# joyecnu/STTODE

Hardware: AMD Instinct MI355X
Metric: predicted-trajectories/sec (20-sample best-of-K) (higher is better)
Workload: dtype f32

## Files before the change

### sttode_amd/csrc/chain32.hip

```cpp
#include "chain.hpp"
#include "latency_bodies.hpp"
#include "frontend_body.hpp"
#include "api_util.hpp"
#include "../../include/sttode_hip.h"
#include <cstdlib>
#include <cstddef>

#ifdef C32_DIAG_TRACE
__shared__ long long g_tr_ph[4];
#define C32_TRACE_BEGIN() long long _tr_t0 = 0, _tr_c0 = 0; if (threadIdx.x == 0 && A.dbg) { _tr_t0 = __builtin_amdgcn_s_memrealtime(); _tr_c0 = __builtin_amdgcn_s_memtime(); }
#define C32_TRACE_END(kind) do { if (threadIdx.x == 0 && A.dbg) { \
        const long long _t1 = __builtin_amdgcn_s_memrealtime(); unsigned _hw, _xcc; \
        asm volatile("s_getreg_b32 %0, hwreg(HW_REG_HW_ID)" : "=s"(_hw)); asm volatile("s_getreg_b32 %0, hwreg(HW_REG_XCC_ID)" : "=s"(_xcc)); \
        const unsigned long long _r = atomicAdd((unsigned long long*)A.dbg, 1ull); if ((long long)_r >= A.dbg[1]) break;  \
        long long* _p = A.dbg + 8 + _r * 12; _p[0] = A.trace_tag; _p[1] = blockIdx.x; _p[2] = (kind); _p[3] = _tr_t0; _p[4] = _t1; _p[5] = _hw; _p[6] = _xcc; \
        _p[8] = g_tr_ph[0]; _p[9] = g_tr_ph[1]; _p[10] = g_tr_ph[2]; _p[7] = __builtin_amdgcn_s_memtime() - _tr_c0; _p[11] = g_tr_ph[3]; } } while (0)
#define C32_TRACE_PHASE(i) do { if (threadIdx.x == 0) g_tr_ph[i] = __builtin_amdgcn_s_memrealtime(); } while (0)
#else
#define C32_TRACE_PHASE(i) do { } while (0)
#define C32_TRACE_BEGIN() do { } while (0)
#define C32_TRACE_END(kind) do { } while (0)
#endif

#include "role_body.hpp"
// ... 186 lines not shown
        asm volatile("s_waitcnt lgkmcnt(0)" ::: "memory");
#endif
        par ^= 1;
        fetched = false;
        __builtin_amdgcn_sched_barrier(0);
    }
};
typedef ChainStreamT<C32_CMAX * C32_TILE, false> ChainStream;

__device__ __forceinline__ void tile_mma(f32x16& acc, const f32x4* __restrict__ t, const f32x16& B) {
#pragma unroll
    for (int g = 0; g < 4; ++g) {
        const f32x4 a = t[g * 64];
#pragma unroll
        for (int r = 0; r < 4; ++r) acc = __builtin_amdgcn_mfma_f32_32x32x2f32(a[r], B[4 * g + r], acc, 0, 0, 0);
    }
}

__device__ __forceinline__ void gather_rows(const void* base, unsigned voff, unsigned slot_addr) {
    glds16_sv<0>(base, voff, slot_addr);
    glds16_sv<32>(base, voff, slot_addr + 1024);
    glds16_sv<64>(base, voff, slot_addr + 2048);
    glds16_sv<96>(base, voff, slot_addr + 3072);
}
__device__ __forceinline__ unsigned row_off(int row, int width, int h) { return (unsigned)row * (unsigned)(width * 4) + (unsigned)h * 16; }

struct Frag { f32x4 a[4]; };
__device__ __forceinline__ void ldfrag(Frag& f, const f32x4* __restrict__ t) {
#pragma unroll
    for (int g = 0; g < 4; ++g) f.a[g] = t[g * 64];
}
__device__ __forceinline__ void tile_mma2(f32x16& acc, const Frag& cur, const f32x16& B, Frag& nxt, const f32x4* __restrict__ tn) {
#pragma unroll
    for (int g = 0; g < 4; ++g) {
        if (g == 2 && tn) {
            ldfrag(nxt, tn);
            __builtin_amdgcn_sched_barrier(0);
        }
#pragma unroll
        for (int r = 0; r < 4; ++r) acc = __builtin_amdgcn_mfma_f32_32x32x2f32(cur.a[g][r], B[4 * g + r], acc, 0, 0, 0);
    }
}

template <class ST>
__device__ __forceinline__ void tile_mma2f(ST& st, f32x16& acc, const Frag& cur, const f32x16& B, Frag& nxt, const f32x4* __restrict__ tn, int nf = 1) {
#pragma unroll
    for (int g = 0; g < 4; ++g) {
        if (g == 2) {
            __builtin_amdgcn_sched_barrier(0);
            if (nf >= 1) st.fetch();
            if (nf >= 2) st.fetch_more();
            if (tn) ldfrag(nxt, tn);
            __builtin_amdgcn_sched_barrier(0);
        }
#pragma unroll
        for (int r = 0; r < 4; ++r) acc = __builtin_amdgcn_mfma_f32_32x32x2f32(cur.a[g][r], B[4 * g + r], acc, 0, 0, 0);
    }
}

template <int KH, class ST>
__device__ __forceinline__ void mlp_l12(ST& st, const f32x4* slot, const f32x4* zslot, const f32x16* Bh, const float* tab, unsigned aoff,
                                        const float* tab_next, unsigned aoff_next, f32x16 (&acc2)[8], int lane) {
    const unsigned slot_addr = __builtin_amdgcn_readfirstlane(lds_addr(slot));
    constexpr int KT1 = 1 + KH;
    static_assert((KT1 + 8) % 3 == 0, "hidden tile must be a whole number of chunks");
#pragma unroll
    for (int R = 0; R < 8; ++R) acc2[R] = splat16(0.f);
#pragma unroll 1
    for (int ht = 0; ht < 16; ++ht) {
        f32x16 h1, zb;
#pragma unroll
        for (int a = 0; a < 4; ++a) {
            const f32x4 v = slot[a * 64 + lane];
            h1[4 * a + 0] = v[0]; h1[4 * a + 1] = v[1]; h1[4 * a + 2] = v[2]; h1[4 * a + 3] = v[3];
        }
#pragma unroll
        for (int a = 0; a < 4; ++a) {
            const f32x4 v = zslot[a * 64 + lane];
            zb[4 * a + 0] = v[0]; zb[4 * a + 1] = v[1]; zb[4 * a + 2] = v[2]; zb[4 * a + 3] = v[3];
        }
        asm volatile("s_waitcnt lgkmcnt(0)" ::: "memory");
        __builtin_amdgcn_sched_barrier(0);
        const bool nl = ht + 1 < 16;
        const void* nb = nl ? (const void*)(reinterpret_cast<const char*>(tab) + 128 * (ht + 1)) : (const void*)tab_next;
        const unsigned no = nl ? aoff : aoff_next;
        Frag fr[2];
#pragma unroll
        for (int i = 0; i < KT1 + 8; ++i) {
            if (i % 3 == 0) {
                if (i > 0) st.end();
                ldfrag(fr[i & 1], st.cur());
                st.begin(3);
                if (i == 0) {
#ifndef C32_DIAG_NOGATHER
                    gather_rows(nb, no, slot_addr);
#endif
                    __builtin_amdgcn_sched_barrier(0);
                }
            }
            const f32x4* tn = (i % 3 < 2) ? st.cur() + (i % 3 + 1) * C32_TILE : nullptr;
            if (i == 0) {
                tile_mma2f(st, h1, fr[i & 1], zb, fr[(i + 1) & 1], tn);
            } else if (i < KT1) {
                if (i % 3 == 0) tile_mma2f(st, h1, fr[i & 1], Bh[i - 1], fr[(i + 1) & 1], tn);
                else tile_mma2(h1, fr[i & 1], Bh[i - 1], fr[(i + 1) & 1], tn);
            } else {
                if (i == KT1) h1 = relu16(h1);
                if (i % 3 == 0) tile_mma2f(st, acc2[i - KT1], fr[i & 1], h1, fr[(i + 1) & 1], tn);
                else tile_mma2(acc2[i - KT1], fr[i & 1], h1, fr[(i + 1) & 1], tn);
            }
        }
        st.end();
    }
}

template <int NO, int NEXT = 0, class ST>
__device__ __forceinline__ void mlp_l3(ST& st, f32x16 (&acc2)[8], const float* __restrict__ b2, const float* __restrict__ b3,
                                       f32x16 (&out)[NO], int h) {
#pragma unroll
    for (int R = 0; R < 8; ++R) {
        STT_FENCE();
        const f32x16 b = ldrows(b2 + 32 * R, h);
        acc2[R] = relu16(acc2[R] + b);
        asm volatile("" : "+v"(acc2[R]));
    }
    STT_FENCE();
#pragma unroll
    for (int o = 0; o < NO; ++o) out[o] = ldrows(b3 + 32 * o, h);
    Frag fr[2];
#pragma unroll
    for (int i = 0; i < 8 * NO; ++i) {
        if (i % 3 == 0) {
            if (i > 0) st.end();
            ldfrag(fr[i & 1], st.cur());
            const int left = 8 * NO - (i + 3);
            st.begin(left >= 3 ? 3 : left > 0 ? left : NEXT);
        }
        const f32x4* tn = (i % 3 < 2 && i + 1 < 8 * NO) ? st.cur() + (i % 3 + 1) * C32_TILE : nullptr;
        if (i % 3 == 0) tile_mma2f(st, out[i / 8], fr[i & 1], acc2[i % 8], fr[(i + 1) & 1], tn);
        else tile_mma2(out[i / 8], fr[i & 1], acc2[i % 8], fr[(i + 1) & 1], tn);
    }
    st.end();
}

typedef __bf16 bf16x8 __attribute__((ext_vector_type(8)));
typedef __bf16 bf16x2 __attribute__((ext_vector_type(2)));
typedef float f32x2v __attribute__((ext_vector_type(2)));
typedef unsigned u32x4v __attribute__((ext_vector_type(4)));
#define C32_TILE_B3 384
#define C32_BUF_B3 (C32_CMAX * C32_TILE_B3)
struct B3 { bf16x8 p[3][2]; };
__device__ __forceinline__ float bf_lo(unsigned u) { return __uint_as_float(u << 16); }
__device__ __forceinline__ float bf_hi(unsigned u) { return __uint_as_float(u & 0xffff0000u); }
__device__ __forceinline__ void split3(const f32x16& x, B3& o) {
#pragma unroll
    for (int kb = 0; kb < 2; ++kb) {
        unsigned hi[4], mi[4], lo[4];
#pragma unroll
        for (int q = 0; q < 4; ++q) {
            const float x0 = x[8 * kb + 2 * q], x1 = x[8 * kb + 2 * q + 1];
            const f32x2v v = {x0, x1};
            hi[q] = __builtin_bit_cast(unsigned, __builtin_convertvector(v, bf16x2));
            const float r0 = x0 - bf_lo(hi[q]), r1 = x1 - bf_hi(hi[q]);
            const f32x2v rv = {r0, r1};
            mi[q] = __builtin_bit_cast(unsigned, __builtin_convertvector(rv, bf16x2));
            const f32x2v qv = {r0 - bf_lo(mi[q]), r1 - bf_hi(mi[q])};
            lo[q] = __builtin_bit_cast(unsigned, __builtin_convertvector(qv, bf16x2));
        }
        const u32x4v H = {hi[0], hi[1], hi[2], hi[3]}, M = {mi[0], mi[1], mi[2], mi[3]}, L = {lo[0], lo[1], lo[2], lo[3]};
        o.p[0][kb] = __builtin_bit_cast(bf16x8, H);
        o.p[1][kb] = __builtin_bit_cast(bf16x8, M);
        o.p[2][kb] = __builtin_bit_cast(bf16x8, L);
    }
}
struct Frag6 { f32x4 a[6]; };
__device__ __forceinline__ void ldfrag6(Frag6& f, const f32x4* __restrict__ t) {
#pragma unroll
    for (int i = 0; i < 6; ++i) f.a[i] = t[i * 64];
}
__device__ __forceinline__ void tile_mma_b3(f32x16& acc, const Frag6& cur, const B3& B, Frag6& nxt, const f32x4* __restrict__ tn) {
#pragma unroll
    for (int kb = 0; kb < 2; ++kb) {
        if (kb == 1 && tn) {
            ldfrag6(nxt, tn);
            __builtin_amdgcn_sched_barrier(0);
        }
        const bf16x8 ah = __builtin_bit_cast(bf16x8, cur.a[kb * 3 + 0]), am = __builtin_bit_cast(bf16x8, cur.a[kb * 3 + 1]),
                     al = __builtin_bit_cast(bf16x8, cur.a[kb * 3 + 2]);
        acc = __builtin_amdgcn_mfma_f32_32x32x16_bf16(al, B.p[0][kb], acc, 0, 0, 0);
        acc = __builtin_amdgcn_mfma_f32_32x32x16_bf16(ah, B.p[2][kb], acc, 0, 0, 0);
        acc = __builtin_amdgcn_mfma_f32_32x32x16_bf16(am, B.p[1][kb], acc, 0, 0, 0);
        acc = __builtin_amdgcn_mfma_f32_32x32x16_bf16(am, B.p[0][kb], acc, 0, 0, 0);
        acc = __builtin_amdgcn_mfma_f32_32x32x16_bf16(ah, B.p[1][kb], acc, 0, 0, 0);
        acc = __builtin_amdgcn_mfma_f32_32x32x16_bf16(ah, B.p[0][kb], acc, 0, 0, 0);
    }
}
__device__ __forceinline__ void tile_mma_b3n(f32x16& acc, const f32x4* __restrict__ t, const B3& B) {
    Frag6 f, dummy;
    ldfrag6(f, t);
    tile_mma_b3(acc, f, B, dummy, nullptr);
}
template <int KH, bool PRE, class ST>
__device__ __forceinline__ void mlp_l12_b3(ST& st, const f32x4* slot, const f32x4* zslot, const f32x16* Bh, const float* tab, unsigned aoff,
                                           const float* tab_next, unsigned aoff_next, f32x16 (&acc2)[8], int lane) {
    const unsigned slot_addr = __builtin_amdgcn_readfirstlane(lds_addr(slot));
    constexpr int KT1 = 1 + KH;
    static_assert((KT1 + 8) % 3 == 0, "hidden tile must be a whole number of chunks");
#pragma unroll
    for (int R = 0; R < 8; ++R) acc2[R] = splat16(0.f);
    B3 Bz;
    if (KH == 0) {
        f32x16 zb;
#pragma unroll
        for (int a = 0; a < 4; ++a) {
            const f32x4 v = zslot[a * 64 + lane];
            zb[4 * a + 0] = v[0]; zb[4 * a + 1] = v[1]; zb[4 * a + 2] = v[2]; zb[4 * a + 3] = v[3];
        }
        split3(zb, Bz);
    }
#pragma unroll 1
    for (int ht = 0; ht < 16; ++ht) {
        f32x16 h1;
#pragma unroll
        for (int a = 0; a < 4; ++a) {
            const f32x4 v = slot[a * 64 + lane];
            h1[4 * a + 0] = v[0]; h1[4 * a + 1] = v[1]; h1[4 * a + 2] = v[2]; h1[4 * a + 3] = v[3];
        }
        B3 Bt;
        if (KH == 0) {
            Bt = Bz;
        } else {
            f32x16 zb;
#pragma unroll
            for (int a = 0; a < 4; ++a) {
                const f32x4 v = zslot[a * 64 + lane];
                zb[4 * a + 0] = v[0]; zb[4 * a + 1] = v[1]; zb[4 * a + 2] = v[2]; zb[4 * a + 3] = v[3];
            }
            split3(zb, Bt);
        }
        asm volatile("s_waitcnt lgkmcnt(0)" ::: "memory");
        __builtin_amdgcn_sched_barrier(0);
        const bool nl = ht + 1 < 16;
        const void* nb = nl ? (const void*)(reinterpret_cast<const char*>(tab) + 128 * (ht + 1)) : (const void*)tab_next;
        const unsigned no = nl ? aoff : aoff_next;
        Frag6 fr[2];
#pragma unroll
        for (int i = 0; i < KT1 + 8; ++i) {
            if (i % 3 == 0) {
                if (i > 0) st.end();
                if (PRE) ldfrag6(fr[i & 1], st.cur());
                st.begin();
                if (i == 0) {
#ifndef C32_DIAG_NOGATHER
                    gather_rows(nb, no, slot_addr);
#endif
                    __builtin_amdgcn_sched_barrier(0);
                }
            }
            const f32x4* tc = st.cur() + (i % 3) * C32_TILE_B3;
            const f32x4* tn = (i % 3 < 2) ? tc + C32_TILE_B3 : nullptr;
            if (i > 0 && i < KT1) {
                STT_FENCE();
                split3(Bh[i - 1], Bt);
            }
            f32x16& acc = i < KT1 ? h1 : acc2[i < KT1 ? 0 : i - KT1];
            if (PRE) tile_mma_b3(acc, fr[i & 1], Bt, fr[(i + 1) & 1], tn);
            else tile_mma_b3n(acc, tc, Bt);
            if (i == KT1 - 1) {
                h1 = relu16(h1);
                split3(h1, Bt);
            }
        }
        st.end();
    }
}
template <int NO, class ST>
__device__ __forceinline__ void mlp_l3_b3(ST& st, f32x16 (&acc2)[8], const float* __restrict__ b2, const float* __restrict__ b3,
                                          f32x16 (&out)[NO], int h) {
#pragma unroll
    for (int o = 0; o < NO; ++o) out[o] = ldrows(b3 + 32 * o, h);
    Frag6 fr[2];
    B3 Bt;
#pragma unroll
    for (int i = 0; i < 8 * NO; ++i) {
        if (i % NO == 0) {
            STT_FENCE();
            const f32x16 b = ldrows(b2 + 32 * (i / NO), h);
            const f32x16 a = relu16(acc2[i / NO] + b);
            split3(a, Bt);
        }
        if (i % 3 == 0) {
            if (i > 0) st.end();
            ldfrag6(fr[i & 1], st.cur());
            st.begin();
        }
        const f32x4* tn = (i % 3 < 2 && i + 1 < 8 * NO) ? st.cur() + (i % 3 + 1) * C32_TILE_B3 : nullptr;
        tile_mma_b3(out[i % NO], fr[i & 1], Bt, fr[(i + 1) & 1], tn);
    }
    st.end();
}

__device__ __forceinline__ f32x16 b3_to_f32(const B3& b) {
    f32x16 r;
#pragma unroll
    for (int kb = 0; kb < 2; ++kb) {
        const u32x4v H = __builtin_bit_cast(u32x4v, b.p[0][kb]), M = __builtin_bit_cast(u32x4v, b.p[1][kb]), L = __builtin_bit_cast(u32x4v, b.p[2][kb]);
#pragma unroll
        for (int q = 0; q < 4; ++q) {
            r[8 * kb + 2 * q] = (bf_lo(H[q]) + bf_lo(M[q])) + bf_lo(L[q]);
            r[8 * kb + 2 * q + 1] = (bf_hi(H[q]) + bf_hi(M[q])) + bf_hi(L[q]);
        }
    }
    return r;
}
template <class ST>
__device__ __forceinline__ void gru32_steps_b3(ST& st, const float* gb, const float* cb, const f32x16& d, f32x16 (&hs)[3], int Tp, int h) {
    B3 dB, hB[3];
    split3(d, dB);
#pragma unroll
    for (int j = 0; j < 3; ++j) split3(hs[j], hB[j]);
    constexpr int T = C32_TILE_B3;
#pragma unroll 1
    for (int t = 0; t < Tp; ++t) {
        B3 eB;
        {
            f32x16 e = ldrows(cb, h);
            st.begin();
            tile_mma_b3n(e, st.cur(), dB);
            e = relu16(e);
            st.end();
            split3(e, eB);
        }
        f32x16 hn[3];
#pragma unroll
        for (int j = 0; j < 3; ++j) {
            STT_FENCE();
            f32x16 ar = ldrows(gb + 0 * 96 + 32 * j, h);
            st.begin();
            tile_mma_b3n(ar, st.cur(), eB);
            tile_mma_b3n(ar, st.cur() + T, hB[0]);
            tile_mma_b3n(ar, st.cur() + 2 * T, hB[1]);
            st.end(); st.begin();
            tile_mma_b3n(ar, st.cur(), hB[2]);
#pragma unroll
            for (int r = 0; r < 16; ++r) ar[r] = C32_SIG(ar[r]);
            STT_FENCE();
            f32x16 az = ldrows(gb + 1 * 96 + 32 * j, h);
            tile_mma_b3n(az, st.cur() + T, eB);
            tile_mma_b3n(az, st.cur() + 2 * T, hB[0]);
            st.end(); st.begin();
            tile_mma_b3n(az, st.cur(), hB[1]);
            tile_mma_b3n(az, st.cur() + T, hB[2]);
#pragma unroll
            for (int r = 0; r < 16; ++r) az[r] = C32_SIG(az[r]);
            STT_FENCE();
            f32x16 an = ldrows(gb + 3 * 96 + 32 * j, h);
            tile_mma_b3n(an, st.cur() + 2 * T, hB[0]);
            st.end(); st.begin();
            tile_mma_b3n(an, st.cur(), hB[1]);
            tile_mma_b3n(an, st.cur() + T, hB[2]);
            {
                const f32x16 bi = ldrows(gb + 2 * 96 + 32 * j, h);
#pragma unroll
                for (int r = 0; r < 16; ++r) an[r] = fmaf(ar[r], an[r], bi[r]);
            }
            STT_FENCE();
            tile_mma_b3n(an, st.cur() + 2 * T, eB);
            st.end();
            const f32x16 hp = b3_to_f32(hB[j]);
#pragma unroll
            for (int r = 0; r < 16; ++r) {
                const float ng = C32_TANH(an[r]);
                hn[j][r] = fmaf(az[r], hp[r] - ng, ng);
            }
        }
#pragma unroll
        for (int j = 0; j < 3; ++j) {
            hs[j] = hn[j];
            split3(hn[j], hB[j]);
        }
    }
}

template <bool ZS, class ST>
__device__ __forceinline__ f32x16 gru32_conv(ST& st, const float* cb, const f32x16& d, int t, int Tp, int h, bool pre) {
    f32x16 e = ldrows(cb, h);
    Frag fa, fb;
    if (ZS) {
        const int k0 = 2 * t - 2, k1 = 2 * t + 3;
        const int g0 = (k0 > 0 ? k0 : 0) >> 3, g1 = (k1 < 2 * Tp - 1 ? k1 : 2 * Tp - 1) >> 3;
        const f32x4* tc = st.cur();
#pragma unroll
        for (int g = 0; g < 4; ++g)
            if (g >= g0 && g <= g1) fa.a[g] = tc[g * 64];
        st.begin(3);
#pragma unroll
        for (int g = 0; g < 4; ++g)
            if (g >= g0 && g <= g1)
#pragma unroll
                for (int r = 0; r < 4; ++r) e = __builtin_amdgcn_mfma_f32_32x32x2f32(fa.a[g][r], d[4 * g + r], e, 0, 0, 0);
        __builtin_amdgcn_sched_barrier(0);
        if (pre) st.take_prefetched();
        else st.fetch();
    } else {
        ldfrag(fa, st.cur());
        st.begin(3);
        tile_mma2f(st, e, fa, d, fb, nullptr, pre ? 0 : 1);
        if (pre) st.take_prefetched();
    }
    e = relu16(e);
    st.end();
    return e;
}

template <bool ZS, class ST>
__device__ __forceinline__ void gru32_steps(ST& st, const float* gb, const float* cb, const f32x16& d, f32x16 (&hs)[3], int Tp, int h) {
    if (ZS) {
        const f32x16 e = gru32_conv<ZS>(st, cb, d, 0, Tp, h, false);
        Frag fa, fb;
#pragma unroll
        for (int j = 0; j < 3; ++j) {
            STT_FENCE();
            f32x16 ar = ldrows(gb + 0 * 96 + 32 * j, h);
            ldfrag(fa, st.cur()); st.begin(3);
            tile_mma2f(st, ar, fa, e, fb, nullptr);
            st.end(); ldfrag(fa, st.cur() + 1 * C32_TILE); st.begin(3);
#pragma unroll
            for (int r = 0; r < 16; ++r) ar[r] = C32_SIG(ar[r]);
            STT_FENCE();
            f32x16 az = ldrows(gb + 1 * 96 + 32 * j, h);
            tile_mma2f(st, az, fa, e, fb, nullptr, 2);
            st.end(); st.begin(3);
            st.take_prefetched();
#pragma unroll
            for (int r = 0; r < 16; ++r) az[r] = C32_SIG(az[r]);
            STT_FENCE();
            f32x16 an = ldrows(gb + 3 * 96 + 32 * j, h);
            {
                const f32x16 bi = ldrows(gb + 2 * 96 + 32 * j, h);
#pragma unroll
                for (int r = 0; r < 16; ++r) an[r] = fmaf(ar[r], an[r], bi[r]);
            }
            st.end(); ldfrag(fa, st.cur() + 2 * C32_TILE);
            if (j < 2) st.begin(3); else st.begin();
            STT_FENCE();
            tile_mma2f(st, an, fa, e, fb, nullptr, (j == 2 && 1 < Tp) ? 2 : 1);
            st.end();
#pragma unroll
            for (int r = 0; r < 16; ++r) {
                const float ng = C32_TANH(an[r]);
                hs[j][r] = fmaf(az[r], 0.f - ng, ng);
            }
        }
    }
#pragma unroll 1
    for (int t = ZS ? 1 : 0; t < Tp; ++t) {
        const f32x16 e = gru32_conv<ZS>(st, cb, d, t, Tp, h, ZS);
        Frag fa, fb;
        f32x16 hn[3];
#pragma unroll
        for (int j = 0; j < 3; ++j) {
            STT_FENCE();
            f32x16 ar = ldrows(gb + 0 * 96 + 32 * j, h);
            ldfrag(fa, st.cur()); st.begin(3);
            tile_mma2f(st, ar, fa, e, fb, st.cur() + 1 * C32_TILE);
            tile_mma2(ar, fb, hs[0], fa, st.cur() + 2 * C32_TILE);
            tile_mma2(ar, fa, hs[1], fb, nullptr);
            st.end(); ldfrag(fa, st.cur()); st.begin(3);
            tile_mma2f(st, ar, fa, hs[2], fb, st.cur() + 1 * C32_TILE);
#pragma unroll
            for (int r = 0; r < 16; ++r) ar[r] = C32_SIG(ar[r]);
            STT_FENCE();
            f32x16 az = ldrows(gb + 1 * 96 + 32 * j, h);
            tile_mma2(az, fb, e, fa, st.cur() + 2 * C32_TILE);
            tile_mma2(az, fa, hs[0], fb, nullptr);
            st.end(); ldfrag(fa, st.cur()); st.begin(3);
            tile_mma2f(st, az, fa, hs[1], fb, st.cur() + 1 * C32_TILE);
            tile_mma2(az, fb, hs[2], fa, st.cur() + 2 * C32_TILE);
#pragma unroll
            for (int r = 0; r < 16; ++r) az[r] = C32_SIG(az[r]);
            STT_FENCE();
            f32x16 an = ldrows(gb + 3 * 96 + 32 * j, h);
            tile_mma2(an, fa, hs[0], fb, nullptr);
            st.end(); ldfrag(fa, st.cur());
            if (j < 2) st.begin(3); else st.begin();
            tile_mma2f(st, an, fa, hs[1], fb, st.cur() + 1 * C32_TILE, (ZS && j == 2 && t + 1 < Tp) ? 2 : 1);
            tile_mma2(an, fb, hs[2], fa, st.cur() + 2 * C32_TILE);
            {
                const f32x16 bi = ldrows(gb + 2 * 96 + 32 * j, h);
#pragma unroll
                for (int r = 0; r < 16; ++r) an[r] = fmaf(ar[r], an[r], bi[r]);
            }
            STT_FENCE();
            tile_mma2(an, fa, e, fb, nullptr);
            st.end();
#pragma unroll
            for (int r = 0; r < 16; ++r) {
                const float ng = C32_TANH(an[r]);
                hn[j][r] = fmaf(az[r], hs[j][r] - ng, ng);
            }
        }
#pragma unroll
        for (int j = 0; j < 3; ++j) hs[j] = hn[j];
    }

}

#include "role32.hpp"

__device__ __forceinline__ int opaque(int v) { asm volatile("" : "+v"(v)); return v; }

#ifdef C32_DIAG_STAMPS
#define C32_STAMP(k) do { if (threadIdx.x == 0 && A.dbg && gi < 4) { A.dbg[((size_t)blockIdx.x * 4 + gi) * 16 + 2 * (k)] = __builtin_amdgcn_s_memtime(); \
                                                                    A.dbg[((size_t)blockIdx.x * 4 + gi) * 16 + 2 * (k) + 1] = __builtin_amdgcn_s_memrealtime(); } } while (0)
#else
#define C32_STAMP(k) do { } while (0)
#endif

__host__ __device__ __forceinline__ int fused_block_of(long b, long T, long G, long K, long lead) {
    auto roles_upto = [&](long x) { const long c = (8 * (x + lead + 1) + K - 1) / K; return c < T ? c : T; };
    long lo = -1, hi = G - 1;
    while (lo < hi) {
        const long mid = (lo + hi + 1) >> 1;
        if (mid + roles_upto(mid) <= b) lo = mid; else hi = mid - 1;
    }
    if (lo >= 0 && lo + roles_upto(lo) == b) return (int)lo;
    return -1 - (int)(b - (lo + 1));
}

__host__ __device__ __forceinline__ int xcd_group(int b, int G) {
    const int x = b & 7, i = b >> 3, q = G >> 3, r = G & 7;
    return x * q + (x < r ? x : r) + i;
}

template <int NY, int FUSE, bool B3M, bool ZS>
__global__ __launch_bounds__(256, 2) void traj_chain_kernel(ChainArgs A) {
    constexpr bool kDynCount = !B3M && ((NY == 1 && FUSE == 2 && !ZS) || (NY == 2 && FUSE == 1 && ZS));
    typedef ChainStreamT<B3M ? C32_BUF_B3 : C32_CMAX * C32_TILE, B3M, kDynCount> Stream;
    extern __shared__ __attribute__((aligned(16))) char smem[];
    f32x4* ring = reinterpret_cast<f32x4*>(smem);
    f32x4* slots = ring + 2 * Stream::kBuf;
    f32x4* zslots = slots + 4 * C32_SLOT;
    float* cst = reinterpret_cast<float*>(zslots + 4 * C32_SLOT);
    int* sq = reinterpret_cast<int*>(cst + C32Const<NY>::total);
    typedef C32Const<NY> CO;

    const int lane = threadIdx.x & 63, c = lane & 31, h = lane >> 5;
    const int wave = __builtin_amdgcn_readfirstlane(threadIdx.x >> 6);
    const f32x4* slot = slots + wave * C32_SLOT;
    const f32x4* zslot = zslots + wave * C32_SLOT;
    const unsigned slot_addr = __builtin_amdgcn_readfirstlane(lds_addr(slot));
    const unsigned zslot_addr = __builtin_amdgcn_readfirstlane(lds_addr(zslot));
    const int ngroups = (A.ncols + 127) >> 7;

    C32_TRACE_BEGIN();
    if (FUSE == 2 && (int)blockIdx.x < A.R32.nwg) {
        role32_body<ZS>(*(KRole32Args*)((const __attribute__((address_space(4))) char*)__builtin_amdgcn_kernarg_segment_ptr() + offsetof(ChainArgs, R32)),
                    blockIdx.x, smem);
        C32_TRACE_END(1);
        return;
    }
    if (FUSE == 1 && A.R.split && (int)blockIdx.x < 5 * A.R.ntiles) {
        split_role(A.R, (A.ncols + A.K - 1) / A.K, A.Tp, A.ldx, A.xpad, blockIdx.x, smem);
        C32_TRACE_END(1);
        return;
    }
    int fb = FUSE == 0 ? (int)blockIdx.x : FUSE == 2 ? (int)blockIdx.x - A.R32.nwg : A.R.split ? (int)blockIdx.x - 5 * A.R.ntiles
                                                : fused_block_of(blockIdx.x, A.R.ntiles, ngroups, A.K, A.R.lead);
    if (FUSE && A.xcd_map && fb >= 0) fb = xcd_group(fb, ngroups);
    if (FUSE == 1 && fb < 0) {
        agent_role(A.R, (A.ncols + A.K - 1) / A.K, A.Tp, A.ldx, A.xpad, -1 - fb, smem);
        C32_TRACE_END(1);
        return;
    }
    for (int i = threadIdx.x; i < CO::total; i += blockDim.x) cst[i] = A.consts[i];
    if (threadIdx.x == 0) sq[0] = FUSE == 2 ? fb : (FUSE == 0 && A.persistent) ? atomicAdd(A.counter, 1) : FUSE ? fb : (int)blockIdx.x;
    if (FUSE == 1) {
        const int g0 = fb;
        const int c_lo = g0 * 128, c_hi = (c_lo + 127 < A.ncols ? c_lo + 127 : A.ncols - 1);
        const int t_lo = (c_lo / A.K) >> 4, t_hi = (c_hi / A.K) >> 4;
        if (wave == 0) {
            const bool ok = A.R.split ? wait_tiles(A.R.pflags, 3 * t_lo, 3 * t_hi + 2, A.R.flags + A.R.ntiles, lane, A.R.tmo_host)
                                      : wait_tiles(A.R.flags, t_lo, t_hi, A.R.flags + A.R.ntiles, lane, A.R.tmo_host);
            if (!ok && lane == 0) sq[0] = -1;
        }
    }
    __syncthreads();
    C32_TRACE_PHASE(3);
    int g = sq[0];
    if (FUSE == 1 && g < 0) {
        for (int i = threadIdx.x; i < 128 * A.Tf2; i += blockDim.x) {
            const size_t o = (size_t)fb * 128 * A.Tf2 + i;
            if (o < (size_t)A.ncols * A.Tf2) A.pred[o] = __builtin_nanf("");
        }
        return;
    }
    if (g >= ngroups) return;
    Stream st;
    st.init(A.pool, A.prog, A.prog_len, ring);

    auto col_of = [&](int gg) { int col = gg * 128 + wave * 32 + c; return col < A.ncols ? col : A.ncols - 1; };
    {
        const int c0 = col_of(g);
        gather_rows(A.A0x, row_off(c0 / A.K, 512, h), slot_addr);
        gather_rows(A.z, row_off(c0, 32, h), zslot_addr);
    }
    asm volatile("s_waitcnt vmcnt(0)" ::: "memory");
    __syncthreads();

    int gi = 0;
    (void)gi;
    while (true) {
        C32_STAMP(0);
        const int col = g * 128 + wave * 32 + c;
        int colc = col < A.ncols ? col : A.ncols - 1;
        int agent = colc / A.K;
        const bool live = col < A.ncols;
        __syncthreads();
        if (threadIdx.x == 0)
            sq[1] = (FUSE == 2 && A.persistent && ngroups > A.nworkers) ? A.nworkers + atomicAdd(A.counter, 1)
                    : (FUSE == 0 && A.persistent) ? atomicAdd(A.counter, 1) : ngroups;

        f32x16 acc2[8];
        f32x16 d;
        {
            agent = opaque(agent);
            f32x16 xo[1];
            const unsigned ao = row_off(agent, 512, h);
            if (B3M) {
                mlp_l12_b3<0, true>(st, slot, zslot, nullptr, A.A0x, ao, A.A0y, ao, acc2, lane);
                mlp_l3_b3<1>(st, acc2, cst + CO::b2x, cst + CO::b3x, xo, h);
            } else {
                mlp_l12<0>(st, slot, zslot, nullptr, A.A0x, ao, A.A0y, ao, acc2, lane);
                mlp_l3<1, 3>(st, acc2, cst + CO::b2x, cst + CO::b3x, xo, h);
            }
            agent = opaque(agent);
            const float* xp = A.xpad + (size_t)agent * A.ldx;
#pragma unroll
            for (int a = 0; a < 4; ++a) {
                f32x4 v = splat4(0.f);
                if (8 * a + 4 * h < A.ldx) v = ld4(xp + 8 * a + 4 * h);
#pragma unroll
                for (int b = 0; b < 4; ++b) d[4 * a + b] = v[b] - xo[0][4 * a + b];
            }
        }
        STT_FENCE();
        C32_STAMP(1);
        {
            agent = opaque(agent);
            f32x16 yo[NY];
            const unsigned ao = row_off(agent, 512, h);
            if (B3M) {
                mlp_l12_b3<0, true>(st, slot, zslot, nullptr, A.A0y, ao, A.A1y, ao, acc2, lane);
                mlp_l3_b3<NY>(st, acc2, cst + CO::b2y, cst + CO::b3y, yo, h);
            } else {
                mlp_l12<0>(st, slot, zslot, nullptr, A.A0y, ao, A.A1y, ao, acc2, lane);
                mlp_l3<NY, 1>(st, acc2, cst + CO::b2y, cst + CO::b3y, yo, h);
            }
            if (live) {
                float* prow = A.park + (size_t)opaque(col) * A.Tf2;
#pragma unroll
                for (int o = 0; o < NY; ++o)
#pragma unroll
                    for (int a = 0; a < 4; ++a) {
                        const int row0 = 32 * o + 8 * a + 4 * h;
                        float* p = prow + row0;
                        if (row0 + 3 < A.Tf2 && (A.Tf2 & 3) == 0) {
                            f32x4 v = {yo[o][4 * a], yo[o][4 * a + 1], yo[o][4 * a + 2], yo[o][4 * a + 3]};
                            st4(p, v);
                        } else {
#pragma unroll
                            for (int b = 0; b < 4; ++b)
                                if (row0 + b < A.Tf2) p[b] = yo[o][4 * a + b];
                        }
                    }
            }
        }
        STT_FENCE();
        C32_STAMP(2);
        f32x16 hs[3];
        {
#pragma unroll
            for (int j = 0; j < 3; ++j) hs[j] = splat16(0.f);
            if (B3M) gru32_steps_b3(st, cst + CO::gb, cst + CO::cb, d, hs, A.Tp, h);
            else gru32_steps<ZS>(st, cst + CO::gb, cst + CO::cb, d, hs, A.Tp, h);
        }
        STT_FENCE();
        C32_STAMP(3);
        const int gnext = sq[1];
        {
            agent = opaque(agent);
            const int cnx = col_of(gnext < ngroups ? gnext : g);
            const unsigned ao = row_off(agent, 512, h), an = row_off(cnx / A.K, 512, h);
            if (B3M) mlp_l12_b3<3, false>(st, slot, zslot, hs, A.A1y, ao, A.A0x, an, acc2, lane);
            else mlp_l12<3>(st, slot, zslot, hs, A.A1y, ao, A.A0x, an, acc2, lane);
            gather_rows(A.z, row_off(opaque(cnx), 32, h), zslot_addr);
            f32x16 yo[NY];
            if (B3M) mlp_l3_b3<NY>(st, acc2, cst + CO::b2m, cst + CO::b3m, yo, h);
            else mlp_l3<NY, 3>(st, acc2, cst + CO::b2m, cst + CO::b3m, yo, h);
            {
                agent = opaque(agent);
                const float cx = A.cur[2 * agent], cy = A.cur[2 * agent + 1];
                const float ox = A.orig[2 * agent], oy = A.orig[2 * agent + 1];
                const bool vec = (A.Tf2 & 3) == 0;
                const float* yrow = A.park + (size_t)opaque(colc) * A.Tf2;
                float* prow = A.pred + (size_t)opaque(col) * A.Tf2;
                const float* grow = FUSE == 2 && A.m_gt ? A.m_gt + (size_t)agent * A.Tf2 : nullptr;
                float dd[NY][4][2];
#pragma unroll
                for (int o = 0; o < NY; ++o)
#pragma unroll
                    for (int a = 0; a < 4; ++a) {
                        const int row0 = 32 * o + 8 * a + 4 * h;
                        const bool whole = vec && row0 + 3 < A.Tf2;
                        f32x4 y0 = splat4(0.f);
                        if (whole) y0 = ld4(yrow + row0);
                        else {
#pragma unroll
                            for (int b = 0; b < 4; ++b)
                                if (row0 + b < A.Tf2) y0[b] = yrow[row0 + b];
                        }
                        f32x4 v;
                        v[0] = ((y0[0] + yo[o][4 * a + 0]) + cx) + ox;
                        v[1] = ((y0[1] + yo[o][4 * a + 1]) + cy) + oy;
                        v[2] = ((y0[2] + yo[o][4 * a + 2]) + cx) + ox;
                        v[3] = ((y0[3] + yo[o][4 * a + 3]) + cy) + oy;
                        if (live) {
                            if (whole) st4(prow + row0, v);
                            else {
#pragma unroll
                                for (int b = 0; b < 4; ++b)
                                    if (row0 + b < A.Tf2) prow[row0 + b] = v[b];
                            }
                        }
                        dd[o][a][0] = dd[o][a][1] = 0.f;
                        if (FUSE == 2 && grow) {
                            if (row0 < A.Tf2) { const float2 g = *reinterpret_cast<const float2*>(grow + row0); dd[o][a][0] = bok_dist(v[0], v[1], g.x, g.y, A.m_scale); }
                            if (row0 + 2 < A.Tf2) { const float2 g = *reinterpret_cast<const float2*>(grow + row0 + 2); dd[o][a][1] = bok_dist(v[2], v[3], g.x, g.y, A.m_scale); }
                        }
                    }
                if (FUSE == 2 && grow) {
                    const int Tf = A.Tf2 >> 1;
                    float acc = 0.f, fdl = -1.f;
#pragma unroll
                    for (int o = 0; o < NY; ++o)
#pragma unroll
                        for (int a = 0; a < 4; ++a) {
                            const int t0 = (32 * o + 8 * a + 4 * h) >> 1;
                            float mine = acc;
                            if (h == 0) { if (t0 < Tf) mine += dd[o][a][0]; if (t0 + 1 < Tf) mine += dd[o][a][1]; }
                            float mine1 = __shfl(mine, c, 64);
                            if (h == 1) { if (t0 < Tf) mine1 += dd[o][a][0]; if (t0 + 1 < Tf) mine1 += dd[o][a][1]; }
                            acc = __shfl(mine1, c + 32, 64);
                            if (t0 == Tf - 1) fdl = dd[o][a][0];
                            if (t0 + 1 == Tf - 1) fdl = dd[o][a][1];
                        }
                    fdl = fmaxf(fdl, __shfl_xor(fdl, 32, 64));
                    const float adev = acc / (float)Tf;
                    if (live && h == 0) {
                        atomicMin(reinterpret_cast<unsigned*>(A.m_ade) + agent, __float_as_uint(adev));
                        atomicMin(reinterpret_cast<unsigned*>(A.m_fde) + agent, __float_as_uint(fdl));
                    }
                }
            }
        }
        C32_STAMP(4);
#ifdef C32_DIAG_STAMPS
        if (threadIdx.x == 0 && A.dbg && gi < 4) {
            long long* o = A.dbg + ((size_t)blockIdx.x * 4 + gi) * 16 + 10;
            o[0] = st.gap_cyc; o[1] = st.gap_n; o[2] = st.gap_cal;
        }
        st.gap_cyc = 0; st.gap_n = 0;
#endif
        ++gi;
        g = gnext;
        if (g >= ngroups) break;
    }
    C32_TRACE_END(0);
}

struct Gru32Args {
    const float* xin; int ldx;
    const f32x4* pool; const int2* prog; int prog_len;
    const float* consts;
    float* state;
    int ncols, Tp;
};
template <bool ZS>
__global__ __launch_bounds__(256, 2) void gru32_kernel(Gru32Args A) {
    extern __shared__ __attribute__((aligned(16))) char smem[];
    f32x4* ring = reinterpret_cast<f32x4*>(smem);
    float* cst = reinterpret_cast<float*>(ring + C32_RING);
    const int lane = threadIdx.x & 63, c = lane & 31, h = lane >> 5;
    const int wave = __builtin_amdgcn_readfirstlane(threadIdx.x >> 6);
    for (int i = threadIdx.x; i < 416; i += blockDim.x) cst[i] = A.consts[i];
    __syncthreads();
    ChainStream st;
    st.init(A.pool, A.prog, A.prog_len, ring);
    const int col = blockIdx.x * 128 + wave * 32 + c;
    const int colc = col < A.ncols ? col : A.ncols - 1;
    f32x16 d;
    {
        const float* xp = A.xin + (size_t)colc * A.ldx;
#pragma unroll
        for (int a = 0; a < 4; ++a) {
            f32x4 v = splat4(0.f);
            if (8 * a + 4 * h < A.ldx) v = ld4(xp + 8 * a + 4 * h);
#pragma unroll
            for (int b = 0; b < 4; ++b) d[4 * a + b] = v[b];
        }
    }
    asm volatile("s_waitcnt vmcnt(0)" ::: "memory");
    __syncthreads();
    f32x16 hs[3];
#pragma unroll
    for (int j = 0; j < 3; ++j) hs[j] = splat16(0.f);
    gru32_steps<ZS>(st, cst, cst + 384, d, hs, A.Tp, h);
    if (col < A.ncols) {
#pragma unroll
        for (int j = 0; j < 3; ++j)
#pragma unroll
            for (int a = 0; a < 4; ++a) {
                const f32x4 v = {hs[j][4 * a], hs[j][4 * a + 1], hs[j][4 * a + 2], hs[j][4 * a + 3]};
                st4(A.state + (size_t)col * 96 + 32 * j + 8 * a + 4 * h, v);
            }
    }
}

static int chain_cus() {
    static int n = 0;
    if (!n) {
        int dev = 0;
        hipDeviceProp_t p;
        if (hipGetDevice(&dev) == hipSuccess && hipGetDeviceProperties(&p, dev) == hipSuccess) n = p.multiProcessorCount;
        if (n <= 0) n = 256;
    }
    return n;
}
static int gru_zero_skip() {
    static const int v = getenv("STTODE_GRU_ZERO_SKIP") ? atoi(getenv("STTODE_GRU_ZERO_SKIP")) != 0 : 1;
    return v;
}
static int chain_lds(int NY, bool b3 = false) { return ((b3 ? 2 * C32_BUF_B3 : C32_RING) + 8 * C32_SLOT) * 16 + (1216 + 64 * NY) * 4 + 16; }

static int role_lds(int Tp) {
    const int e = (Tp * 256 + 512) * 16, g = (2 * 6 * 64 + 2 * 24 * 64 + 2 * 4 * 64) * 16;
    return e > g ? e : g;
// ... 283 lines not shown
```

Baseline: 86.79 million.

## Skip zero-hidden and zero-band MFMA work in bf16x3 GRU steps

Restructures the bf16x3 GRU recurrence into a per-step template. The first step is specialised for a zero hidden state, which drops all hidden-state MFMAs, and in the ZS mode each k-block of the conv input product is skipped when its band is empty. The lane-half row offset is now computed inside the kernel from mbcnt instead of being passed as h, and the gather offsets are adjusted to match. The goal is to remove redundant matrix-core work and splitting on zero operands, at the cost of more template code and a risk of subtle offset bugs.

New measurement: 86.81 million (median of 3 runs). No clear change (+0.0%).

```diff
diff --git a/sttode_amd/csrc/chain32.hip b/sttode_amd/csrc/chain32.hip
--- a/sttode_amd/csrc/chain32.hip
+++ b/sttode_amd/csrc/chain32.hip
@@ -362,26 +362,32 @@
 struct B3 { bf16x8 p[3][2]; };
 __device__ __forceinline__ float bf_lo(unsigned u) { return __uint_as_float(u << 16); }
 __device__ __forceinline__ float bf_hi(unsigned u) { return __uint_as_float(u & 0xffff0000u); }
+__device__ __forceinline__ void split3_kb(const f32x16& x, B3& o, int kb) {
+    unsigned hi[4], mi[4], lo[4];
+#pragma unroll
+    for (int q = 0; q < 4; ++q) {
+        const float x0 = x[8 * kb + 2 * q], x1 = x[8 * kb + 2 * q + 1];
+        const f32x2v v = {x0, x1};
+        hi[q] = __builtin_bit_cast(unsigned, __builtin_convertvector(v, bf16x2));
+        const float r0 = x0 - bf_lo(hi[q]), r1 = x1 - bf_hi(hi[q]);
+        const f32x2v rv = {r0, r1};
+        mi[q] = __builtin_bit_cast(unsigned, __builtin_convertvector(rv, bf16x2));
+        const f32x2v qv = {r0 - bf_lo(mi[q]), r1 - bf_hi(mi[q])};
+        lo[q] = __builtin_bit_cast(unsigned, __builtin_convertvector(qv, bf16x2));
+    }
+    const u32x4v H = {hi[0], hi[1], hi[2], hi[3]}, M = {mi[0], mi[1], mi[2], mi[3]}, L = {lo[0], lo[1], lo[2], lo[3]};
+    o.p[0][kb] = __builtin_bit_cast(bf16x8, H);
+    o.p[1][kb] = __builtin_bit_cast(bf16x8, M);
+    o.p[2][kb] = __builtin_bit_cast(bf16x8, L);
+}
 __device__ __forceinline__ void split3(const f32x16& x, B3& o) {
-#pragma unroll
-    for (int kb = 0; kb < 2; ++kb) {
-        unsigned hi[4], mi[4], lo[4];
-#pragma unroll
-        for (int q = 0; q < 4; ++q) {
-            const float x0 = x[8 * kb + 2 * q], x1 = x[8 * kb + 2 * q + 1];
-            const f32x2v v = {x0, x1};
-            hi[q] = __builtin_bit_cast(unsigned, __builtin_convertvector(v, bf16x2));
-            const float r0 = x0 - bf_lo(hi[q]), r1 = x1 - bf_hi(hi[q]);
-            const f32x2v rv = {r0, r1};
-            mi[q] = __builtin_bit_cast(unsigned, __builtin_convertvector(rv, bf16x2));
-            const f32x2v qv = {r0 - bf_lo(mi[q]), r1 - bf_hi(mi[q])};
-            lo[q] = __builtin_bit_cast(unsigned, __builtin_convertvector(qv, bf16x2));
-        }
-        const u32x4v H = {hi[0], hi[1], hi[2], hi[3]}, M = {mi[0], mi[1], mi[2], mi[3]}, L = {lo[0], lo[1], lo[2], lo[3]};
-        o.p[0][kb] = __builtin_bit_cast(bf16x8, H);
-        o.p[1][kb] = __builtin_bit_cast(bf16x8, M);
-        o.p[2][kb] = __builtin_bit_cast(bf16x8, L);
-    }
+    split3_kb(x, o, 0);
+    split3_kb(x, o, 1);
+}
+__device__ __forceinline__ int lane_half() {
+    int l = __builtin_amdgcn_mbcnt_hi(~0u, __builtin_amdgcn_mbcnt_lo(~0u, 0u));
+    asm volatile("" : "+v"(l));
+    return l >> 5;
 }
 struct Frag6 { f32x4 a[6]; };
 __device__ __forceinline__ void ldfrag6(Frag6& f, const f32x4* __restrict__ t) {
@@ -452,7 +458,7 @@
         __builtin_amdgcn_sched_barrier(0);
         const bool nl = ht + 1 < 16;
         const void* nb = nl ? (const void*)(reinterpret_cast<const char*>(tab) + 128 * (ht + 1)) : (const void*)tab_next;
-        const unsigned no = nl ? aoff : aoff_next;
+        const unsigned no = (nl ? aoff : aoff_next) + (KH ? (unsigned)lane_half() << 4 : 0u);
         Frag6 fr[2];
 #pragma unroll
         for (int i = 0; i < KT1 + 8; ++i) {
@@ -523,72 +529,99 @@
     }
     return r;
 }
-template <class ST>
+__device__ __forceinline__ void tile_kb_b3(f32x16& acc, const f32x4* __restrict__ t, const B3& B, int kb) {
+    const bf16x8 ah = __builtin_bit_cast(bf16x8, t[(kb * 3 + 0) * 64]), am = __builtin_bit_cast(bf16x8, t[(kb * 3 + 1) * 64]),
+                 al = __builtin_bit_cast(bf16x8, t[(kb * 3 + 2) * 64]);
+    acc = __builtin_amdgcn_mfma_f32_32x32x16_bf16(al, B.p[0][kb], acc, 0, 0, 0);
+    acc = __builtin_amdgcn_mfma_f32_32x32x16_bf16(ah, B.p[2][kb], acc, 0, 0, 0);
+    acc = __builtin_amdgcn_mfma_f32_32x32x16_bf16(am, B.p[1][kb], acc, 0, 0, 0);
+    acc = __builtin_amdgcn_mfma_f32_32x32x16_bf16(am, B.p[0][kb], acc, 0, 0, 0);
+    acc = __builtin_amdgcn_mfma_f32_32x32x16_bf16(ah, B.p[1][kb], acc, 0, 0, 0);
+    acc = __builtin_amdgcn_mfma_f32_32x32x16_bf16(ah, B.p[0][kb], acc, 0, 0, 0);
+}
+template <bool ZS, bool H0, class ST>
+__device__ __forceinline__ void gru32_step_b3(ST& st, const float* gb, const float* cb, const f32x16& d, B3 (&hB)[3], f32x16 (&hs)[3], int t, int Tp) {
+    constexpr int T = C32_TILE_B3;
+    B3 eB;
+    {
+        f32x16 e = ldrows(cb, lane_half());
+        B3 dB;
+        st.begin();
+        if (ZS) {
+            const int c0 = 2 * t - 2 > 0 ? 2 * t - 2 : 0, c1 = 2 * t + 3 < 2 * Tp - 1 ? 2 * t + 3 : 2 * Tp - 1;
+            if (c0 <= 15) { split3_kb(d, dB, 0); tile_kb_b3(e, st.cur(), dB, 0); }
+            if (c1 >= 16) { split3_kb(d, dB, 1); tile_kb_b3(e, st.cur(), dB, 1); }
+        } else {
+            split3(d, dB);
+            tile_mma_b3n(e, st.cur(), dB);
+        }
+        e = relu16(e);
+        st.end();
+        split3(e, eB);
+    }
+    f32x16 hn[3];
+#pragma unroll
+    for (int j = 0; j < 3; ++j) {
+        STT_FENCE();
+        f32x16 ar = ldrows(gb + 0 * 96 + 32 * j, lane_half());
+        st.begin();
+        tile_mma_b3n(ar, st.cur(), eB);
+        if (!H0) tile_mma_b3n(ar, st.cur() + T, hB[0]);
+        if (!H0) tile_mma_b3n(ar, st.cur() + 2 * T, hB[1]);
+        st.end(); st.begin();
+        if (!H0) tile_mma_b3n(ar, st.cur(), hB[2]);
+#pragma unroll
+        for (int r = 0; r < 16; ++r) ar[r] = C32_SIG(ar[r]);
+        STT_FENCE();
+        f32x16 az = ldrows(gb + 1 * 96 + 32 * j, lane_half());
+        tile_mma_b3n(az, st.cur() + T, eB);
+        if (!H0) tile_mma_b3n(az, st.cur() + 2 * T, hB[0]);
+        st.end(); st.begin();
+        if (!H0) tile_mma_b3n(az, st.cur(), hB[1]);
+        if (!H0) tile_mma_b3n(az, st.cur() + T, hB[2]);
+#pragma unroll
+        for (int r = 0; r < 16; ++r) az[r] = C32_SIG(az[r]);
+        STT_FENCE();
+        f32x16 an = ldrows(gb + 3 * 96 + 32 * j, lane_half());
+        if (!H0) tile_mma_b3n(an, st.cur() + 2 * T, hB[0]);
+        st.end(); st.begin();
+        if (!H0) tile_mma_b3n(an, st.cur(), hB[1]);
+        if (!H0) tile_mma_b3n(an, st.cur() + T, hB[2]);
+        {
+            const f32x16 bi = ldrows(gb + 2 * 96 + 32 * j, lane_half());
+#pragma unroll
+            for (int r = 0; r < 16; ++r) an[r] = fmaf(ar[r], an[r], bi[r]);
+        }
+        STT_FENCE();
+        tile_mma_b3n(an, st.cur() + 2 * T, eB);
+        st.end();
+        const f32x16 hp = H0 ? splat16(0.f) : b3_to_f32(hB[j]);
+#pragma unroll
+        for (int r = 0; r < 16; ++r) {
+            const float ng = C32_TANH(an[r]);
+            hn[j][r] = fmaf(az[r], hp[r] - ng, ng);
+        }
+    }
+#pragma unroll
+    for (int j = 0; j < 3; ++j) {
+        hs[j] = hn[j];
+        split3(hn[j], hB[j]);
+    }
+}
+template <bool ZS, class ST>
 __device__ __forceinline__ void gru32_steps_b3(ST& st, const float* gb, const float* cb, const f32x16& d, f32x16 (&hs)[3], int Tp, int h) {
-    B3 dB, hB[3];
-    split3(d, dB);
-#pragma unroll
-    for (int j = 0; j < 3; ++j) split3(hs[j], hB[j]);
-    constexpr int T = C32_TILE_B3;
+    B3 hB[3];
+    f32x16 dd = d;
+    if (ZS) {
+        gru32_step_b3<true, true>(st, gb, cb, dd, hB, hs, 0, Tp);
+    } else {
+#pragma unroll
+        for (int j = 0; j < 3; ++j) split3(hs[j], hB[j]);
+    }
 #pragma unroll 1
-    for (int t = 0; t < Tp; ++t) {
-        B3 eB;
-        {
-            f32x16 e = ldrows(cb, h);
-            st.begin();
-            tile_mma_b3n(e, st.cur(), dB);
-            e = relu16(e);
-            st.end();
-            split3(e, eB);
-        }
-        f32x16 hn[3];
-#pragma unroll
-        for (int j = 0; j < 3; ++j) {
-            STT_FENCE();
-            f32x16 ar = ldrows(gb + 0 * 96 + 32 * j, h);
-            st.begin();
-            tile_mma_b3n(ar, st.cur(), eB);
-            tile_mma_b3n(ar, st.cur() + T, hB[0]);
-            tile_mma_b3n(ar, st.cur() + 2 * T, hB[1]);
-            st.end(); st.begin();
-            tile_mma_b3n(ar, st.cur(), hB[2]);
-#pragma unroll
-            for (int r = 0; r < 16; ++r) ar[r] = C32_SIG(ar[r]);
-            STT_FENCE();
-            f32x16 az = ldrows(gb + 1 * 96 + 32 * j, h);
-            tile_mma_b3n(az, st.cur() + T, eB);
-            tile_mma_b3n(az, st.cur() + 2 * T, hB[0]);
-            st.end(); st.begin();
-            tile_mma_b3n(az, st.cur(), hB[1]);
-            tile_mma_b3n(az, st.cur() + T, hB[2]);
-#pragma unroll
-            for (int r = 0; r < 16; ++r) az[r] = C32_SIG(az[r]);
-            STT_FENCE();
-            f32x16 an = ldrows(gb + 3 * 96 + 32 * j, h);
-            tile_mma_b3n(an, st.cur() + 2 * T, hB[0]);
-            st.end(); st.begin();
-            tile_mma_b3n(an, st.cur(), hB[1]);
-            tile_mma_b3n(an, st.cur() + T, hB[2]);
-            {
-                const f32x16 bi = ldrows(gb + 2 * 96 + 32 * j, h);
-#pragma unroll
-                for (int r = 0; r < 16; ++r) an[r] = fmaf(ar[r], an[r], bi[r]);
-            }
-            STT_FENCE();
-            tile_mma_b3n(an, st.cur() + 2 * T, eB);
-            st.end();
-            const f32x16 hp = b3_to_f32(hB[j]);
-#pragma unroll
-            for (int r = 0; r < 16; ++r) {
-                const float ng = C32_TANH(an[r]);
-                hn[j][r] = fmaf(az[r], hp[r] - ng, ng);
-            }
-        }
-#pragma unroll
-        for (int j = 0; j < 3; ++j) {
-            hs[j] = hn[j];
-            split3(hn[j], hB[j]);
-        }
+    for (int t = ZS ? 1 : 0; t < Tp; ++t) {
+        asm volatile("" : "+v"(dd));
+        gru32_step_b3<ZS, false>(st, gb, cb, dd, hB, hs, t, Tp);
     }
 }
 
@@ -892,7 +925,7 @@
         {
 #pragma unroll
             for (int j = 0; j < 3; ++j) hs[j] = splat16(0.f);
-            if (B3M) gru32_steps_b3(st, cst + CO::gb, cst + CO::cb, d, hs, A.Tp, h);
+            if (B3M) gru32_steps_b3<ZS>(st, cst + CO::gb, cst + CO::cb, d, hs, A.Tp, h);
             else gru32_steps<ZS>(st, cst + CO::gb, cst + CO::cb, d, hs, A.Tp, h);
         }
         STT_FENCE();
@@ -902,7 +935,7 @@
             agent = opaque(agent);
             const int cnx = col_of(gnext < ngroups ? gnext : g);
             const unsigned ao = row_off(agent, 512, h), an = row_off(cnx / A.K, 512, h);
-            if (B3M) mlp_l12_b3<3, false>(st, slot, zslot, hs, A.A1y, ao, A.A0x, an, acc2, lane);
+            if (B3M) mlp_l12_b3<3, false>(st, slot, zslot, hs, A.A1y, row_off(agent, 512, 0), A.A0x, row_off(cnx / A.K, 512, 0), acc2, lane);
             else mlp_l12<3>(st, slot, zslot, hs, A.A1y, ao, A.A0x, an, acc2, lane);
             gather_rows(A.z, row_off(opaque(cnx), 32, h), zslot_addr);
             f32x16 yo[NY];
```
